# TejasPote/data_diet_distributed

Hardware: AMD Instinct MI355X
Metric: examples scored/sec (whole node), EL2N+GraNd ResNet-18 CIFAR-10, 1/2/4/8 GPU (higher is better)
Workload: dtype fp32 (split MFMA: hi*hi + hi*lo + lo*hi with fp32 accumulation; EL2N forward on f16x3 halves, GraNd forward on f16x3, GraNd backward on bf16x3); 1 GPU; R18/C10 EL2N+GraNd, K checkpoints, global keep-set; arch=resnet18, input=3x32x32 cifar stem, n_examples=50000, checkpoints=10, classes=10, score_batch=128, grand_batch=1024, el2n_chunk=1024, kept=25000, select_by=el2n, pegrad_method=auto, grand_params=conv_linear, passes=sequential, lanes=3, launch_plan=full chunks + short tail, el2n_operands=f16x3

## Files before the change

data_diet_distributed_amd/csrc/dd_conv_kern.h:

```cpp
#pragma once

#ifndef DD_R2_FENCE
#define DD_R2_FENCE 2
#endif
#include "dd_mfma.h"

namespace dd {
namespace conv {

struct Args {
  const float* x;
  const __bf16* wpack;
  const float* bias;
  const float* residual;
  const float* mask_src;
  const float* in_scale;
  const float* in_shift;
  float* y;
  float* stats;
  uint16_t* mask_out;
  const uint16_t* mask_in;
  int64_t B, n_stat;
  int cin, H, cout, op, cp;
  int relu, xf_mask, gsize, tiles_per_group;
// ... 60 lines not shown
  static constexpr int XS = W * 2;
  static constexpr int PLANE = CC * XS;
  static constexpr int ROWP = 3 * 2 * PLANE + (W == 16 ? 128 : W == 8 ? 64 : W == 4 ? 32 : 0);
  static constexpr int IMGP = (RB + 2) * ROWP + (W == 4 ? 192 : 0);
  static constexpr int BUF = E * IMGP;
  static constexpr int LDS = 2 * BUF > BUF + 16384 ? 2 * BUF : BUF + 16384;
  static constexpr int TB = E * RB * W;
  static constexpr int TW = TB / WT;
  static constexpr int NT = TW / 32;
  static constexpr int OB = WO * NA * 32;
  static constexpr int TPR = W / 4;
  static constexpr int NF4 = NR * CC * W / 4;
  static constexpr int NST = (NF4 + 255) / 256;
  static_assert(TW % 32 == 0 && NT >= 1, "a wave must own whole 32-position tiles");
  static_assert(WO * WT == 4, "four waves per workgroup");
};

template <int W, int RB, int E, int NA, int WO, int XF, bool KX1, int EPI = 0, int PW = 0>
__global__ __launch_bounds__(256, NA == 1 ? 2 : 1) void conv3x3_kernel(const Args A) {
  using C = Cfg<W, RB, E, NA, WO>;
  constexpr int NT = C::NT;
  constexpr bool F16 = (EPI & kEpiF16) != 0;
  static_assert(!PW || (XF <= kXfAffine && !KX1 && (EPI & ~kEpiF16) == (kEpiSpec | kEpiStats)),
                "padded-width tiles: the statistics epilogue with an optional BN staging only");
  extern __shared__ __attribute__((aligned(16))) char smem[];
  const int H = A.H, cin = A.cin, cout = A.cout;
  const int64_t B = A.B;
  const float* __restrict__ x = A.x;
  const int WG = PW ? A.wg : W;
  const int HW = H * WG;
// ... 453 lines not shown
      }
    }
    for (; kc + 1 < nchunks; ++kc) chunk(T, kc + 1, true);
    const Tile Tn = has_next ? decode(tile_n) : T;
    chunk(Tn, has_next ? 0 : nchunks - 1, false);
    load_w_taps(Tn.ob32, 0, 0, 3);
    epilogue(T, tile, (g - 1) & 1);
    __syncthreads();
    load_w_taps(Tn.ob32, 0, 3, 6);
    if (!has_next) break;
    tile = tile_n;
    T = Tn;
  }
}

template <int W, int RB, int E, int WO, int XF, bool KX1, int EPI = 0, int PW = 0>
__global__ __launch_bounds__(256, 2) void conv3x3_r2_kernel(const Args A) {
  using C = Cfg<W, RB, E, 1, WO>;
  constexpr int NT = C::NT;
  constexpr bool F16 = (EPI & kEpiF16) != 0;
  static_assert(!PW || (XF <= kXfAffine && !KX1 && (EPI & ~kEpiF16) == (kEpiSpec | kEpiStats)),
                "padded-width tiles: the statistics epilogue with an optional BN staging only");
  extern __shared__ __attribute__((aligned(16))) char smem[];
  const int H = A.H, cin = A.cin, cout = A.cout;
  const int64_t B = A.B;
  const float* __restrict__ x = A.x;
  const int WG = PW ? A.wg : W;
  const int HW = H * WG;
  const int HWP = PW ? A.n_tb * RB * W : HW;
  const int ntiles = A.n_tiles;

  const int tid = threadIdx.x, lane = tid & 63;
  const int wv = __builtin_amdgcn_readfirstlane(tid >> 6);
  const int wo = wv % WO, wt = wv / WO, h = lane >> 5;

  struct Tile {
    int64_t b, grp;
    int tb, o0, y0, xf_base, ob32;
  };
  auto decode = [&](int tile) {
    Tile T;
    int bid = tile;
    const int ob = bid % A.n_ob;
    bid /= A.n_ob;
    T.tb = bid % A.n_tb;
    T.b = (int64_t)(bid / A.n_tb) * E;
    T.o0 = ob * C::OB;
    T.y0 = T.tb * RB;
    T.grp = T.b / A.gsize;
    T.xf_base = (int)(T.grp * cin);
    T.ob32 = (T.o0 >> 5) + wo;
    return T;
  };

  float4 ra[C::NST];
  static_assert(256 % (C::TPR * CC) == 0, "a thread's staged channel must not depend on k");
  float xs = 1.f, xt = 0.f;
  bool va[C::NST];
  float4 rv[C::NST];
  float rs = 1.f, rt = 0.f;
  __amdgpu_buffer_rsrc_t xo_rsrc;
  int xo_base = 0;
  bool xo_tile = false;
  auto load_chunk = [&](const Tile& T, int c0) {
    const int64_t left = (B - T.b) * cin * HW * 4;
    const uint32_t range = (uint32_t)(left < 0x7fffffff ? left : 0x7fffffff);
    const __amdgpu_buffer_rsrc_t xr = buffer_rsrc(x + (size_t)T.b * cin * HW, range);
    const int ubase = c0 * HW * 4;
    __amdgpu_buffer_rsrc_t rr_rsrc;
    if constexpr (XF >= kXfOut) {
      xo_rsrc = buffer_rsrc(A.xout + (size_t)T.b * cin * HW, range);
      xo_base = ubase + (T.y0 - 1) * W * 4;
      xo_tile = T.o0 == 0;
      if constexpr (XF >= kXfOutRes) rr_rsrc = buffer_rsrc(A.xres + (size_t)T.b * cin * HW, range);
    }
#pragma unroll
    for (int k = 0; k < C::NST; ++k) {
      const int q = tid + 256 * k;
      const int x4 = q % C::TPR, c = (q / C::TPR) % CC, sr = q / (C::TPR * CC);
      const int e = sr / (RB + 2), rr = sr - e * (RB + 2);
      const int ir = T.y0 - 1 + rr, cg = c0 + c;
      va[k] = q < C::NF4 && ir >= 0 && ir < H && cg < cin && T.b + e < B &&
              (!PW || x4 * 4 < WG);
      const int irc = ir < 0 ? 0 : (ir >= H ? H - 1 : ir);
      const int xoff = ubase + ((e * cin + c) * HW + irc * WG + x4 * 4) * 4;
      if constexpr (PW == 2) {
        ra[k] = make_float4(
            __builtin_bit_cast(float, __builtin_amdgcn_raw_buffer_load_b32(xr, xoff, 0, 0)),
            __builtin_bit_cast(float, __builtin_amdgcn_raw_buffer_load_b32(xr, xoff + 4, 0, 0)),
            __builtin_bit_cast(float, __builtin_amdgcn_raw_buffer_load_b32(xr, xoff + 8, 0, 0)),
            __builtin_bit_cast(float, __builtin_amdgcn_raw_buffer_load_b32(xr, xoff + 12, 0, 0)));
      } else {
        ra[k] = __builtin_bit_cast(float4, __builtin_amdgcn_raw_buffer_load_b128(xr, xoff, 0, 0));
// ... 5 lines not shown
    }
    if constexpr (XF != kXfNone) {
      const int cg = c0 + (tid / C::TPR) % CC;
      const int xi = T.xf_base + (cg < cin ? cg : cin - 1);
      xs = A.in_scale[xi];
      xt = A.in_shift[xi];
      if constexpr (XF == kXfOutResAff) {
        rs = A.xres_scale[xi];
        rt = A.xres_shift[xi];
      }
    }
  };
  auto store_chunk = [&](int buf) {
    char* base0 = smem + buf * C::BUF;
#pragma unroll
    for (int k = 0; k < C::NST; ++k) {
      const int q = tid + 256 * k;
      if (C::NF4 % 256 != 0 && k == C::NST - 1 && q >= C::NF4) continue;
      const int x4 = q % C::TPR, c = (q / C::TPR) % CC, sr = q / (C::TPR * CC);
      const int se = sr / (RB + 2), rr = sr - se * (RB + 2);
      float4 v = ra[k];
      if constexpr (XF != kXfNone) v = stage_transform<XF>(v, xs, xt, rv[k], rs, rt, A.in_floor);
      v = keep_if(v, va[k]);
      if constexpr (PW == 2) v = keep_cols(v, WG - x4 * 4);
      if constexpr (XF >= kXfOut) {
        const bool wr = xo_tile && va[k] && rr >= 1 && rr <= RB;
        const int off = xo_base + ((se * cin + c) * HW + rr * W + x4 * 4) * 4;
        __builtin_amdgcn_raw_buffer_store_b128(__builtin_bit_cast(uint4v, v), xo_rsrc,
                                               wr ? off : (int)0x80000000, 0, 0);
      }
      uint2 hs[3], ls[3];
      split_shift3<F16>(v, x4 == 0, x4 == C::TPR - 1, hs, ls);
      if constexpr (KX1) {
// ... 57 lines not shown
    floatx16 d = acc[n];
    d = mfma16<F16>(ws[set][kx][0], bb[n][0], d);
    d = mfma16<F16>(ws[set][kx][0], bb[n][1], d);
    d = mfma16<F16>(ws[set][kx][1], bb[n][0], d);
    acc[n] = d;
  };

  auto epilogue = [&](const Tile& T, int tile, int free_buf) {
    const EpiFlags F = epi_flags<EPI>(A);
    const float* __restrict__ bias = A.bias;
    const float* __restrict__ residual = A.residual;
    const float* __restrict__ mask_src = A.mask_src;
    float* __restrict__ y = A.y;
    float* ep = reinterpret_cast<float*>(smem + free_buf * C::BUF) + wv * 1024;
    const int tl = lane & 7, ol = lane >> 3;
    size_t ibase[NT];
    bool vlan[NT];
    float in_stat[NT];
    int ncol[NT];
#pragma unroll
    for (int n = 0; n < NT; ++n) {
      const int tt = wt * C::TW + n * 32 + 4 * tl;
      const int e = tt / (RB * W);
      int t = T.y0 * W + tt % (RB * W);
      bool in_img = true;
      if constexpr (PW) {
        const int rem = tt % (RB * W), row = T.y0 + rem / W, col = rem % W;
        in_img = row < H && col < WG;
        ncol[n] = WG - col;
        t = in_img ? row * WG + col : 0;
// ... 32 lines not shown
      if (F.msrc) {
#pragma unroll
        for (int m = 0; m < NG; ++m) {
          unsigned mb = 0;
#pragma unroll
          for (int k = 0; k < 4; ++k) {
            const float4 mk = *reinterpret_cast<const float4*>(mask_src + ibase[n0 + m] + off[k]);
            mb |= ((mk.x > 0.f ? 1u : 0u) | (mk.y > 0.f ? 2u : 0u) | (mk.z > 0.f ? 4u : 0u) |
                   (mk.w > 0.f ? 8u : 0u)) << (4 * k);
          }
          mbits[m] = mb;
        }
      } else {
#pragma unroll
        for (int m = 0; m < NG; ++m) {
          const size_t fidx = (((size_t)tile * 4 + wv) * NT + n0 + m) * 64 + lane;
          mbits[m] = F.min ? A.mask_in[fidx] : 0xffffu;
        }
      }
#pragma unroll
      for (int m = 0; m < NG; ++m) {
        const int n = n0 + m;
#pragma unroll
        for (int r = 0; r < 16; ++r)
          ep[((r & 3) + 8 * (r >> 2) + 4 * h) * 32 + (lane & 31)] =
              F16 ? acc[n][r] * A.acc_scale : acc[n][r];
        asm volatile("" ::: "memory");
        float4 v[4];
#pragma unroll
        for (int k = 0; k < 4; ++k)
          v[k] = *reinterpret_cast<const float4*>(ep + (8 * k + ol) * 32 + 4 * tl);
// ... 31 lines not shown
#pragma unroll
              for (int j = 0; j < 4; ++j)
                if (j < ncol[n]) y[ibase[n] + off[k] + j] = f[j];
            }
          } else if (vlan[n] && o < cout) {
            store_out4(y + ibase[n] + off[k], f[0], f[1], f[2], f[3]);
          }
          if (F.stats) {
            s_ = sum8(s_);
            q_ = sum8(q_);
            if (tl == 0 && o < cout)
              *reinterpret_cast<float2*>(sp + k * 16 * A.tiles_per_group) = make_float2(s_, q_);
          }
        }
        if (F.mout) {
          const size_t fidx = (((size_t)tile * 4 + wv) * NT + n) * 64 + lane;
          A.mask_out[fidx] = (uint16_t)obits;
        }
      }
    });
  };

  auto chunk = [&](auto Pc, auto W2c, const Tile& T, int c, const Tile& Ts, int ks,
                   const Tile& Tw, int kw) {
    constexpr int P = decltype(Pc)::value;
    load_chunk(Ts, ks * CC);
#if DD_R2_FENCE >= 1
    __builtin_amdgcn_sched_barrier(0);
#endif
    constexpr int T0 = KX1 ? 1 : 0, TS = KX1 ? 3 : 1;
#pragma unroll
// ... 141 lines not shown

template <int W, int RB, int E, int NA, int WO>
struct GoNarrow {
  const Args& a;
  dim3 g;
  hipStream_t st;
  template <int XF, bool KX1, int EPI>
  int run() {
    constexpr auto K = &conv3x3_kernel<W, RB, E, NA, WO, XF, KX1, EPI>;
    lds_attr<K>(Cfg<W, RB, E, NA, WO>::LDS);
    K<<<g, 256, Cfg<W, RB, E, NA, WO>::LDS, st>>>(a);
    DD_CHECK_LAUNCH("dd_conv3x3_forward");
    return DD_OK;
  }
};
template <int W, int RB, int E, int WO>
struct GoR2 {
  static constexpr int LDS = Cfg<W, RB, E, 1, WO>::LDS;
  const Args& a;
  dim3 g;
  hipStream_t st;
  template <int XF, bool KX1, int EPI>
  int run() {
    constexpr auto K = &conv3x3_r2_kernel<W, RB, E, WO, XF, KX1, EPI>;
    lds_attr<K>(LDS);
    K<<<g, 256, LDS, st>>>(a);
    DD_CHECK_LAUNCH("dd_conv3x3_forward");
    return DD_OK;
  }
};

template <int W, int RB, int E, int NA, int WO>
static int launch(Args a, hipStream_t st) {
  using C = Cfg<W, RB, E, NA, WO>;
  DD_REQUIRE(a.H % RB == 0, "dd_conv3x3_forward: H must be a multiple of the row block");
  DD_REQUIRE(a.gsize % E == 0, "dd_conv3x3_forward: group_size %d must be a multiple of %d "
             "(images per tile at %dx%d)", a.gsize, E, a.H, W);
  DD_REQUIRE(a.op % C::OB == 0, "dd_conv3x3_forward: padded outputs %d not a multiple of %d",
             a.op, C::OB);
  a.n_tb = a.H / RB;
  a.n_ob = a.op / C::OB;
  const int64_t ntiles = ceil_div(a.B, E) * a.n_tb * a.n_ob;
  DD_REQUIRE(ntiles < (1ll << 31), "dd_conv3x3_forward: too many tiles");
  a.n_tiles = (int)ntiles;
  const int64_t cap = NA == 2 ? device_cus() : a.cin <= 256 ? 2ll * device_cus() : ntiles;
  const int64_t grid = ntiles < cap ? ntiles : cap;
  GoNarrow<W, RB, E, NA, WO> go{a, dim3((unsigned)grid), st};
  return dispatch_epi<kSpecNarrow<W, RB, E, NA, WO>>(a, go);
}

template <int W, int RB, int E, int WO>
static int launch_r2(Args a, hipStream_t st) {
  using C = Cfg<W, RB, E, 1, WO>;
  static_assert(2 * C::LDS <= 160 * 1024, "r2 tiles run two workgroups per CU");
  DD_REQUIRE(a.H % RB == 0, "dd_conv3x3_forward: H must be a multiple of the row block");
  DD_REQUIRE(a.gsize % E == 0, "dd_conv3x3_forward: group_size %d must be a multiple of %d "
             "(images per tile at %dx%d)", a.gsize, E, a.H, W);
  DD_REQUIRE(a.op % C::OB == 0, "dd_conv3x3_forward: padded outputs %d not a multiple of %d",
             a.op, C::OB);
  a.n_tb = a.H / RB;
  a.n_ob = a.op / C::OB;
  const int64_t ntiles = ceil_div(a.B, E) * a.n_tb * a.n_ob;
  DD_REQUIRE(ntiles < (1ll << 31), "dd_conv3x3_forward: too many tiles");
  a.n_tiles = (int)ntiles;
  const int64_t cap = 2ll * device_cus();
  GoR2<W, RB, E, WO> go{a, dim3((unsigned)(ntiles < cap ? ntiles : cap)), st};
  return dispatch_epi<true, decltype(go), W >= 8>(a, go);
}

template <int W, int RB, int E, int PW, int XF, int EPI>
static int run_pw(const Args& a, dim3 g, hipStream_t st) {
  constexpr auto K = &conv3x3_r2_kernel<W, RB, E, 4, XF, false, EPI, PW>;
  lds_attr<K>(Cfg<W, RB, E, 1, 4>::LDS);
  K<<<g, 256, Cfg<W, RB, E, 1, 4>::LDS, st>>>(a);
  DD_CHECK_LAUNCH("dd_conv3x3_forward");
  return DD_OK;
}
template <int W, int RB, int E, int PW>
static int launch_r2_pw(Args a, hipStream_t st) {
  using C = Cfg<W, RB, E, 1, 4>;
  static_assert(2 * C::LDS <= 160 * 1024, "r2 tiles run two workgroups per CU");
// ... 44 lines not shown
  a.n_ob = a.op / C::OB;
  const int64_t ntiles = ceil_div(a.B, E) * a.n_tb * a.n_ob;
  DD_REQUIRE(ntiles < (1ll << 31), "dd_conv3x3_forward: too many tiles");
  a.n_tiles = (int)ntiles;
  const int64_t cap = (int64_t)(160 * 1024 / C::LDS) * device_cus();
  const dim3 g((unsigned)(ntiles < cap ? ntiles : cap));
  const bool xf = a.xf_mask != 0;
  if (a.f16)
    return xf ? run_pw_narrow<W, RB, E, PW, kXfAffine, kE_Stats | kEpiF16>(a, g, st)
              : run_pw_narrow<W, RB, E, PW, kXfNone, kE_Stats | kEpiF16>(a, g, st);
  return xf ? run_pw_narrow<W, RB, E, PW, kXfAffine, kE_Stats>(a, g, st)
            : run_pw_narrow<W, RB, E, PW, kXfNone, kE_Stats>(a, g, st);
}

int dispatch_r2(int w, int key, const Args& a, hipStream_t st);
int dispatch_small(int w, int key, const Args& a, hipStream_t st);
int dispatch_pw(int w, int pw, const Args& a, hipStream_t st);

}
}
```

data_diet_distributed_amd/csrc/dd_conv_r2.hip:

```cpp
#include "dd_conv_kern.h"

namespace dd {
namespace conv {

int dispatch_r2(int w, int k, const Args& a, hipStream_t st) {
  if (w == 16 && k == 8000 + 100 + 10 + 4) return launch_r2<16, 8, 1, 4>(a, st);
  if (w == 8 && k == 8000 + 200 + 10 + 4) return launch_r2<8, 8, 2, 4>(a, st);
  if (w == 4 && k == 4000 + 800 + 10 + 4) return launch_r2<4, 4, 8, 4>(a, st);
  set_error("dd_conv3x3_forward: no r2 kernel for tile key %d at w=%d", k, w);
  return DD_EINVAL;
}

}
}
```

data_diet_distributed_amd/csrc/dd_down.hip:

```cpp
#include "dd_mfma.h"

#include <stdlib.h>

namespace dd {
namespace down {

using namespace conv;

template <int WO, int RB, int E>
struct DCfg {
  static constexpr int SR = 2 * RB + 1;
  static constexpr int NR = E * SR;
  static constexpr int WI = 2 * WO;
  static constexpr int XS = WO * 2;
  static constexpr int PLANE = CC * XS;
  static constexpr int ROWP = 3 * 2 * PLANE + (WO == 16 ? 64 : WO == 8 ? 32 : WO == 4 ? 16 : 0);
  static constexpr int IMGP = SR * ROWP + (WO == 4 ? 240 : 0);
  static constexpr int BUF = E * IMGP;
  static constexpr int TB = E * RB * WO;
  static constexpr int TPR = WI / 8;
  static constexpr int NF8 = NR * CC * WI / 8;
  static constexpr int NST = (NF8 + 255) / 256;
  static constexpr int TPR4 = WI / 4;
  static constexpr int NF4 = NR * CC * WI / 4;
  static constexpr int NST4 = (NF4 + 255) / 256;
  static constexpr int TAILB = (NF8 % 256 != 0 || NF4 % 256 != 0) ? 6 * PLANE + 512 : 0;
  static constexpr int LDS = 2 * BUF + TAILB;
  static_assert(TB == 64, "two 32-position t tiles per workgroup");
  static_assert(WO % 4 == 0, "transposed reads take 4 consecutive columns");
  static_assert(BUF >= 4 * 4096, "the epilogue's four 4 KB transpose blocks live in a buffer");
};

struct Out {
  float* y;
  const float* bias;
  float* stats;
  int relu;
  float scale;
};

struct FwdArgs {
  const float* x;
  const __bf16* w3;
  const __bf16* ws;
  Out main, sc;
  int64_t B, n_stat;
  int cin, HO, cout, nob32;
  int gsize, tiles_per_group, n_tb, n_ob, n_tiles;
  int xcd;
  int wog;
  const float* in_scale;
  const float* in_shift;
  const float* xres;
};

constexpr int kXmNone = 0, kXmAffine = 1, kXmUnit = 3;

template <int WO, int RB, int E, bool SC, bool PT, int WA, int EPI = 0, int XM = 0,
          bool F16 = false, int PW = 0>
__global__ __launch_bounds__(256, 2) void down_fwd_kernel(const FwdArgs A) {
  using C = DCfg<WO, RB, E>;
  constexpr int NT = WA == 4 ? 2 : 1;
  constexpr bool S8 = WO >= 8;
  static_assert(!PW || (!SC && S8 && E == 1 && XM != kXmUnit && EPI == 0),
                "padded-width heads: the plain EL2N statistics launch");
  extern __shared__ __attribute__((aligned(16))) char smem[];
  const int HO = A.HO, HI = 2 * HO, cin = A.cin, cout = A.cout;
  const int64_t B = A.B;
  const int WOG = PW ? A.wog : WO, WIG = 2 * WOG;
  const int HWI = HI * WIG, HWO = HO * WOG;
  const int ntiles = A.n_tiles;

  const int tid = threadIdx.x, lane = tid & 63;
  const int wv = WA == 4 ? __builtin_amdgcn_readfirstlane(tid >> 6) : tid >> 6;
  const int wo = WA == 4 ? wv : wv & 1, wt = WA == 4 ? 0 : wv >> 1, h = lane >> 5;

  struct Tile {
    int64_t b, grp;
    int tb, y0, o_w, ob32;
  };
  auto decode = [&](int tile) {
    Tile T;
    int bid = tile;
    const int ob = bid % A.n_ob;
    bid /= A.n_ob;
    T.tb = bid % A.n_tb;
    T.b = (int64_t)(bid / A.n_tb) * E;
    T.y0 = T.tb * RB;
    T.grp = T.b / A.gsize;
    T.o_w = ob * 32 * WA + wo * 32;
    T.ob32 = T.o_w >> 5;
    return T;
  };

  const float* __restrict__ x = A.x;
  float4 ra4[S8 ? 1 : C::NST4];
  bool va4[S8 ? 1 : C::NST4];
  static_assert(256 % (C::TPR4 * CC) == 0 && 256 % (C::TPR * CC) == 0,
                "a thread's staged channel must not depend on the round");
  float xs = 1.f, xt = 0.f;
  float4 rr4[(S8 || XM != kXmUnit) ? 1 : C::NST4];
  float4 rr8[(S8 && XM == kXmUnit) ? C::NST : 1][2];
  auto load_affine = [&](const Tile& T, int c0, int tpr) {
    if constexpr (XM != kXmNone) {
      const int cg = c0 + (tid / tpr) % CC;
      const int xi = (int)(T.grp * cin) + (cg < cin ? cg : cin - 1);
      xs = A.in_scale[xi];
      xt = A.in_shift[xi];
    }
  };
  auto xform = [&](float4 v, float4 r) {
    if constexpr (XM == kXmNone) {
      return v;
    } else {
      v = make_float4(fmaf(v.x, xs, xt), fmaf(v.y, xs, xt), fmaf(v.z, xs, xt), fmaf(v.w, xs, xt));
      if constexpr (XM == kXmUnit) v = make_float4(v.x + r.x, v.y + r.y, v.z + r.z, v.w + r.w);
      return make_float4(nmax(v.x, 0.f), nmax(v.y, 0.f), nmax(v.z, 0.f), nmax(v.w, 0.f));
    }
  };
  auto load_chunk4 = [&](const Tile& T, int c0) {
#pragma unroll
    for (int k = 0; k < C::NST4; ++k) {
      const int q = tid + 256 * k;
      const int x4 = q % C::TPR4, c = (q / C::TPR4) % CC, sr = q / (C::TPR4 * CC);
      const int e = sr / C::SR, rr = sr - e * C::SR;
      const int ir = 2 * T.y0 - 1 + rr, cg = c0 + c;
      const bool ve = T.b + e < B;
      va4[k] = q < C::NF4 && ir >= 0 && ir < HI && cg < cin && ve;
      const int irc = ir < 0 ? 0 : (ir >= HI ? HI - 1 : ir);
      const int cgc = cg < cin ? cg : cin - 1;
      const int64_t bc = ve ? T.b + e : B - 1;
      const size_t ofs = ((size_t)bc * cin + cgc) * HWI + irc * C::WI + x4 * 4;
      ra4[k] = *reinterpret_cast<const float4*>(x + ofs);
      if constexpr (!S8 && XM == kXmUnit) rr4[k] = *reinterpret_cast<const float4*>(A.xres + ofs);
    }
    load_affine(T, c0, C::TPR4);
  };
  auto store_chunk4 = [&](int buf) {
    char* base0 = smem + buf * C::BUF;
#pragma unroll
    for (int k = 0; k < C::NST4; ++k) {
      const int q = tid + 256 * k;
      const bool tail = C::NF4 % 256 != 0 && k == C::NST4 - 1 && q >= C::NF4;
      const int x4 = q % C::TPR4, c = (q / C::TPR4) % CC, sr = q / (C::TPR4 * CC);
      float4 rk = make_float4(0.f, 0.f, 0.f, 0.f);
      if constexpr (!S8 && XM == kXmUnit) rk = rr4[k];
      const float4 v = keep_if(xform(ra4[k], rk), va4[k]);
      float left = lane_prev<C::TPR4>(v.w);
      if (x4 == 0) left = 0.f;
      const float f[3][2] = {{left, v.y}, {v.x, v.z}, {v.y, v.w}};
#pragma unroll
      for (int kx = 0; kx < 3; ++kx) {
        __bf16 h0, l0, h1, l1;
        split16<F16>(f[kx][0], h0, l0);
        split16<F16>(f[kx][1], h1, l1);
        const int se = sr / C::SR, rr = sr - se * C::SR;
        char* p = tail ? smem + 2 * C::BUF + (kx * 2) * C::PLANE + lane * 4
                       : base0 + se * C::IMGP + rr * C::ROWP + (kx * 2) * C::PLANE + c * C::XS +
                             x4 * 4;
        typedef __bf16 bf16x2 __attribute__((ext_vector_type(2)));
        *reinterpret_cast<bf16x2*>(p) = bf16x2{h0, h1};
        *reinterpret_cast<bf16x2*>(p + C::PLANE) = bf16x2{l0, l1};
      }
    }
  };

  float4 ra[S8 ? C::NST : 1][2];
  bool va[S8 ? C::NST : 1];
  auto load_chunk8 = [&](const Tile& T, int c0) {
#pragma unroll
    for (int k = 0; k < C::NST; ++k) {
      const int q = tid + 256 * k;
      const int x8 = q % C::TPR, c = (q / C::TPR) % CC, sr = q / (C::TPR * CC);
      const int e = sr / C::SR, rr = sr - e * C::SR;
      const int ir = 2 * T.y0 - 1 + rr, cg = c0 + c;
      const bool ve = T.b + e < B;
      va[k] = q < C::NF8 && ir >= 0 && ir < HI && cg < cin && ve && (!PW || x8 * 8 < WIG);
      const int irc = ir < 0 ? 0 : (ir >= HI ? HI - 1 : ir);
      const int cgc = cg < cin ? cg : cin - 1;
      const int64_t bc = ve ? T.b + e : B - 1;
      const int col = PW && x8 * 8 >= WIG ? 0 : x8 * 8;
      const size_t ofs = ((size_t)bc * cin + cgc) * HWI + irc * WIG + col;
      if constexpr (PW == 3) {
        float v[8];
#pragma unroll
        for (int j = 0; j < 8; ++j) v[j] = x[ofs + (col + j < WIG ? j : 0)];
        ra[k][0] = make_float4(v[0], v[1], v[2], v[3]);
// ... 1 lines not shown
      } else {
        ra[k][0] = *reinterpret_cast<const float4*>(x + ofs);
        ra[k][1] = *reinterpret_cast<const float4*>(x + ofs + (!PW || col + 4 < WIG ? 4 : 0));
      }
      if constexpr (S8 && XM == kXmUnit) {
        rr8[k][0] = *reinterpret_cast<const float4*>(A.xres + ofs);
        rr8[k][1] = *reinterpret_cast<const float4*>(A.xres + ofs + 4);
      }
    }
    load_affine(T, c0, C::TPR);
  };
  auto store_chunk8 = [&](int buf) {
    char* base0 = smem + buf * C::BUF;
#pragma unroll
    for (int k = 0; k < C::NST; ++k) {
      const int q = tid + 256 * k;
      const bool tail = C::NF8 % 256 != 0 && k == C::NST - 1 && q >= C::NF8;
      const int x8 = q % C::TPR, c = (q / C::TPR) % CC, sr = q / (C::TPR * CC);
      float4 r0 = make_float4(0.f, 0.f, 0.f, 0.f), r1 = r0;
      if constexpr (S8 && XM == kXmUnit) {
        r0 = rr8[k][0];
        r1 = rr8[k][1];
      }
      float4 v0 = keep_if(xform(ra[k][0], r0), va[k]), v1 = keep_if(xform(ra[k][1], r1), va[k]);
      if constexpr (PW != 0) {
        v0 = keep_cols(v0, WIG - x8 * 8);
        v1 = keep_cols(v1, WIG - x8 * 8 - 4);
      }
      float left = C::TPR > 1 ? lane_prev<C::TPR>(v1.w) : 0.f;
      if (x8 == 0) left = 0.f;
      const float f[9] = {left, v0.x, v0.y, v0.z, v0.w, v1.x, v1.y, v1.z, v1.w};
      __bf16 hv[9], lv[9];
// ... 196 lines not shown
            acc_s[n] = s_;
          }
          if constexpr (t + 1 < 9) rb(t + 1, n);
        }
        if (wload) {
          load_w_taps(Tp.ob32, kn, t, 1);
          if constexpr (t == 4) load_w_sc(Tp.ob32, kn);
        }
        if constexpr (t == 6) store_chunk(cur ^ 1);
        __builtin_amdgcn_sched_barrier(0);
      });
      __syncthreads();
      ++g;
    };
    auto chunk = [&](const Tile& Tp, int kn, bool wload) {
      if constexpr (WA == 4) {
        chunk4(Tp, kn, wload);
        return;
      }
      const int cur = g & 1;
      load_chunk(Tp, kn * CC);
      const char* base = smem + cur * C::BUF;
      bf16x8 b0[3][2], b1[3][2];
      read_b(base, 0, b0);
      __builtin_amdgcn_sched_barrier(0);
      read_b(base, 1, b1);
      mfma_row(0, b0);
      if (wload) load_w_taps(Tp.ob32, kn, 0, 3);
#pragma unroll
      for (int i = 0; i < 3; ++i) {
        __builtin_amdgcn_sched_group_barrier(0x008, 1, 0);
// ... 26 lines not shown
#pragma unroll
      for (int i = 0; i < 9; ++i) {
        __builtin_amdgcn_sched_group_barrier(0x008, 1, 2);
        __builtin_amdgcn_sched_group_barrier(0x002, 5, 2);
        __builtin_amdgcn_sched_group_barrier(0x080, 1, 2);
      }
      __builtin_amdgcn_sched_barrier(0);
      __syncthreads();
      ++g;
    };
    for (int kc = 0; kc + 1 < nchunks; ++kc) chunk(T, kc + 1, true);
    {
      const Tile Tn = has_next ? decode(tile_n) : T;
      chunk(Tn, has_next ? 0 : nchunks - 1, false);
    }
    char* ep_buf = smem + ((g - 1) & 1) * C::BUF;
#pragma unroll
    for (int n = 0; n < NT; ++n) {
      epilogue(T, acc[n], A.main, T.o_w, ep_buf, wt + n, std::true_type{});
      if constexpr (SC) epilogue(T, acc_s[n], A.sc, T.o_w, ep_buf, wt + n, std::false_type{});
    }
    if constexpr (!PT) break;
    __syncthreads();
    const int tile_w = has_next ? tile_n : tile;
    T = decode(tile_w);
    load_w_ordered(T.ob32, 0);
    if (!has_next) break;
    tile = tile_n;
  }
}

// ... 460 lines not shown
    const int no = tflip ? cin : cout, nc = tflip ? cout : cin;
    float v = 0.f;
    if (o < no && c < nc) v = tflip ? w[(size_t)c * cin + o] : w[(size_t)o * cin + c];
    v *= scale;
    __bf16 hi, lo;
    if (f16)
      split16<true>(v, hi, lo);
    else
      split16<false>(v, hi, lo);
    out[i] = pr == 0 ? hi : lo;
  }
}

template <int WO, int RB, int E, bool SC, int WA, int EPI = 0, int XM = 0, bool F16 = false>
static int launch_fwd(FwdArgs a, hipStream_t st) {
  using C = DCfg<WO, RB, E>;
  static bool attr = false;
  if (!attr) {
    (void)hipFuncSetAttribute(
        reinterpret_cast<const void*>(&down_fwd_kernel<WO, RB, E, SC, false, WA, EPI, XM, F16>),
        hipFuncAttributeMaxDynamicSharedMemorySize, C::LDS);
    (void)hipFuncSetAttribute(
        reinterpret_cast<const void*>(&down_fwd_kernel<WO, RB, E, SC, true, WA, EPI, XM, F16>),
        hipFuncAttributeMaxDynamicSharedMemorySize, C::LDS);
    attr = true;
  }
  DD_REQUIRE(a.HO % RB == 0, "dd_down_forward: HO must be a multiple of the row block");
  DD_REQUIRE(a.gsize % E == 0, "dd_down_forward: group_size %d must be a multiple of %d",
             a.gsize, E);
  a.n_tb = a.HO / RB;
  a.n_ob = (int)ceil_div(a.cout, 32 * WA);
  a.tiles_per_group = (a.gsize / E) * a.n_tb * 2;
  const int64_t ntiles = ceil_div(a.B, E) * a.n_tb * a.n_ob;
  DD_REQUIRE(ntiles < (1ll << 31), "dd_down_forward: too many tiles");
  a.n_tiles = (int)ntiles;
  const bool pt = a.cin <= 64;
  const int64_t cap = pt ? 2ll * device_cus() : ntiles;
  const int64_t grid = ntiles < cap ? ntiles : cap;
  if (pt)
    down_fwd_kernel<WO, RB, E, SC, true, WA, EPI, XM, F16>
        <<<(unsigned)grid, 256, C::LDS, st>>>(a);
  else
    down_fwd_kernel<WO, RB, E, SC, false, WA, EPI, XM, F16>
        <<<(unsigned)grid, 256, C::LDS, st>>>(a);
  DD_CHECK_LAUNCH("dd_down_forward");
  return DD_OK;
}

template <int WO, int RB, int PW, int XM, bool F16>
static int launch_fwd_pw(FwdArgs a, hipStream_t st) {
  using C = DCfg<WO, RB, 1>;
  constexpr auto K = &down_fwd_kernel<WO, RB, 1, false, false, 4, 0, XM, F16, PW>;
  static bool attr = false;
  if (!attr) {
    (void)hipFuncSetAttribute(reinterpret_cast<const void*>(K),
                              hipFuncAttributeMaxDynamicSharedMemorySize, C::LDS);
    attr = true;
  }
  a.n_tb = (a.HO + RB - 1) / RB;
// ... 5 lines not shown
  K<<<(unsigned)ntiles, 256, C::LDS, st>>>(a);
  DD_CHECK_LAUNCH("dd_down_forward");
  return DD_OK;
}

static int fwd_epi(const Out& m, const Out& s) {
  static const int f = env_int("DD_DOWN_EPI", 1);
  if (f == 0 || !s.y) return 0;
  if (!m.bias && !m.relu && m.stats && !s.bias && !s.relu && s.stats) return 1;
  if (m.bias && m.relu && !m.stats && s.bias && !s.relu && !s.stats) return 2;
  return 0;
}
static int fwd_wa(int cout) {
  static const int f = env_int("DD_DOWN_WA", 4);
  return f == 4 && conv::pad_to(cout, 64) % 128 == 0 ? 4 : 2;
}

template <int WO, int RB, int E, bool SC>
static int launch_bwd(BwdArgs a, hipStream_t st) {
  using C = UCfg<WO, RB, E, SC>;
  static bool attr = false;
  if (!attr) {
    (void)hipFuncSetAttribute(reinterpret_cast<const void*>(&down_bwd_kernel<WO, RB, E, SC>),
                              hipFuncAttributeMaxDynamicSharedMemorySize, C::LDS);
    attr = true;
  }
  DD_REQUIRE(a.HO % RB == 0, "dd_down_backward: HO must be a multiple of the row block");
  a.n_tb = a.HO / RB;
  a.n_ob = (int)ceil_div(a.cin, 64);
  const int64_t grid = ceil_div(a.B, E) * a.n_tb * a.n_ob;
// ... 173 lines not shown
               "dd_down_forward_unit_input: the unit form needs the fused shortcut and "
               "statistics on both outputs");
    DD_REQUIRE(!in_scale || xres || !sc,
               "dd_down_forward_unit_input: BN + ReLU staging without a shortcut only");
#define DD_DOWN_F(WO_, RB_, E_, WA_)                                                          \
    if (xres) return down::launch_fwd<WO_, RB_, E_, true, WA_, 1, down::kXmUnit, true>(a, st); \
    if (in_scale) return down::launch_fwd<WO_, RB_, E_, false, WA_, 0, down::kXmAffine, true>(a, st); \
    if (sc && epi == 1) return down::launch_fwd<WO_, RB_, E_, true, WA_, 1, 0, true>(a, st); \
    if (sc && epi == 2) return down::launch_fwd<WO_, RB_, E_, true, WA_, 2, 0, true>(a, st); \
    if (sc) return down::launch_fwd<WO_, RB_, E_, true, WA_, 0, 0, true>(a, st);           \
    return down::launch_fwd<WO_, RB_, E_, false, WA_, 0, 0, true>(a, st);
#define DD_DOWN_FW(WO_, RB_, E_) \
    if (wa == 4) { DD_DOWN_F(WO_, RB_, E_, 4) } else { DD_DOWN_F(WO_, RB_, E_, 2) }
    if (wo == 32) { DD_DOWN_FW(32, 2, 1) }
    if (wo == 16) { DD_DOWN_FW(16, 4, 1) }
    if (wo == 8) { DD_DOWN_FW(8, 8, 1) }
    DD_DOWN_FW(4, 4, 4)
#undef DD_DOWN_FW
#undef DD_DOWN_F
  }
  if (in_scale) {
    const int wa = down::fwd_wa(cout);
#define DD_DOWN_X(WO_, RB_, E_)                                                          \
    if (xres) {                                                                          \
      DD_REQUIRE(sc && down::fwd_epi(a.main, a.sc) == 1,                                 \
                 "dd_down_forward_unit_input: the unit form needs the fused shortcut and " \
                 "statistics on both outputs");                                          \
      return wa == 4 ? down::launch_fwd<WO_, RB_, E_, true, 4, 1, down::kXmUnit>(a, st) \
                     : down::launch_fwd<WO_, RB_, E_, true, 2, 1, down::kXmUnit>(a, st); \
    }                                                                                    \
    DD_REQUIRE(!sc, "dd_down_forward_unit_input: BN + ReLU staging without a shortcut only"); \
    return wa == 4 ? down::launch_fwd<WO_, RB_, E_, false, 4, 0, down::kXmAffine>(a, st) \
                   : down::launch_fwd<WO_, RB_, E_, false, 2, 0, down::kXmAffine>(a, st);
    if (wo == 32) { DD_DOWN_X(32, 2, 1) }
    if (wo == 16) { DD_DOWN_X(16, 4, 1) }
    if (wo == 8) { DD_DOWN_X(8, 8, 1) }
    DD_DOWN_X(4, 4, 4)
#undef DD_DOWN_X
  }
  const int wa = down::fwd_wa(cout);
  const int epi = down::fwd_epi(a.main, a.sc);
#define DD_DOWN_SC(WO_, RB_, E_, WA_)                                                  \
  (epi == 1   ? down::launch_fwd<WO_, RB_, E_, true, WA_, 1>(a, st)                \
   : epi == 2 ? down::launch_fwd<WO_, RB_, E_, true, WA_, 2>(a, st)                \
              : down::launch_fwd<WO_, RB_, E_, true, WA_, 0>(a, st))
#define DD_DOWN(WO_, RB_, E_)                                                    \
  return wa == 4 ? (sc ? DD_DOWN_SC(WO_, RB_, E_, 4)                             \
                       : down::launch_fwd<WO_, RB_, E_, false, 4>(a, st))        \
                 : (sc ? DD_DOWN_SC(WO_, RB_, E_, 2)                             \
                       : down::launch_fwd<WO_, RB_, E_, false, 2>(a, st))
  if (wo == 32) DD_DOWN(32, 2, 1);
  if (wo == 16) DD_DOWN(16, 4, 1);
  if (wo == 8) DD_DOWN(8, 8, 1);
  DD_DOWN(4, 4, 4);
#undef DD_DOWN
#undef DD_DOWN_SC
}

int dd_down_forward(const float* x, int64_t B, int32_t cin, int32_t ho, int32_t wo,
                    const void* packed3x3, const void* packed1x1, int32_t cout,
                    const float* bias, int32_t relu, float* stats, float* y,
                    const float* bias_sc, int32_t relu_sc, float* stats_sc, float* y_sc,
                    int32_t group_size, int64_t n_stat, int32_t operands, float acc_scale,
                    float acc_scale_sc, void* stream) {
  clear_error();
  return down_forward_impl(x, B, cin, ho, wo, packed3x3, packed1x1, cout, bias, relu, stats, y,
                           bias_sc, relu_sc, stats_sc, y_sc, group_size, n_stat, nullptr,
// ... 81 lines not shown
```

Before: 8930 examples/s.

## Add 8-wave workgroup variants for small-spatial r2 conv and downsample kernels

Adds 512-thread, eight-wave forms of the r2 3x3 convolution kernel (8x8 and 4x4 maps) and the downsample forward kernel. Each workgroup now spans 256 output channels instead of 128, so one staged input tile is reused across twice as many outputs. Occupancy drops to one workgroup per CU with a larger LDS budget. The mask index math is generalised to the new output blocking. Both forms are on by default through environment flags when cout padding allows it, which risks lower latency hiding and fewer workgroups on the small late layers.

```diff
diff --git a/data_diet_distributed_amd/csrc/dd_conv_kern.h b/data_diet_distributed_amd/csrc/dd_conv_kern.h
--- a/data_diet_distributed_amd/csrc/dd_conv_kern.h
+++ b/data_diet_distributed_amd/csrc/dd_conv_kern.h
@@ -98,6 +98,14 @@
   static constexpr int NST = (NF4 + 255) / 256;
   static_assert(TW % 32 == 0 && NT >= 1, "a wave must own whole 32-position tiles");
   static_assert(WO * WT == 4, "four waves per workgroup");
+};
+
+template <int W, int RB, int E>
+struct R2W8 {
+  using C = Cfg<W, RB, E, 1, 4>;
+  static constexpr int OB = 8 * 32;
+  static constexpr int NST = (C::NF4 + 511) / 512;
+  static constexpr int LDS = 2 * C::BUF > C::BUF + 32768 ? 2 * C::BUF : C::BUF + 32768;
 };
 
 template <int W, int RB, int E, int NA, int WO, int XF, bool KX1, int EPI = 0, int PW = 0>
@@ -581,10 +589,17 @@
   }
 }
 
-template <int W, int RB, int E, int WO, int XF, bool KX1, int EPI = 0, int PW = 0>
-__global__ __launch_bounds__(256, 2) void conv3x3_r2_kernel(const Args A) {
+template <int W, int RB, int E, int WO, int XF, bool KX1, int EPI = 0, int PW = 0, int NW = 4>
+__global__ __launch_bounds__(NW * 64, NW == 4 ? 2 : 1) void conv3x3_r2_kernel(const Args A) {
   using C = Cfg<W, RB, E, 1, WO>;
+  using C8 = R2W8<W, RB, E>;
   constexpr int NT = C::NT;
+  constexpr int NTH = NW * 64;
+  constexpr int WOK = NW == 8 ? 8 : WO;
+  constexpr int OBK = NW == 8 ? C8::OB : C::OB;
+  constexpr int NST = NW == 8 ? C8::NST : C::NST;
+  static_assert(NW == 4 || (NW == 8 && WO == 4 && !PW && !KX1),
+                "the 8-wave form: the native 8x8 / 4x4 tiles, eight waves along o");
   constexpr bool F16 = (EPI & kEpiF16) != 0;
   static_assert(!PW || (XF <= kXfAffine && !KX1 && (EPI & ~kEpiF16) == (kEpiSpec | kEpiStats)),
                 "padded-width tiles: the statistics epilogue with an optional BN staging only");
@@ -599,7 +614,7 @@
 
   const int tid = threadIdx.x, lane = tid & 63;
   const int wv = __builtin_amdgcn_readfirstlane(tid >> 6);
-  const int wo = wv % WO, wt = wv / WO, h = lane >> 5;
+  const int wo = wv % WOK, wt = wv / WOK, h = lane >> 5;
 
   struct Tile {
     int64_t b, grp;
@@ -612,7 +627,7 @@
     bid /= A.n_ob;
     T.tb = bid % A.n_tb;
     T.b = (int64_t)(bid / A.n_tb) * E;
-    T.o0 = ob * C::OB;
+    T.o0 = ob * OBK;
     T.y0 = T.tb * RB;
     T.grp = T.b / A.gsize;
     T.xf_base = (int)(T.grp * cin);
@@ -620,11 +635,11 @@
     return T;
   };
 
-  float4 ra[C::NST];
-  static_assert(256 % (C::TPR * CC) == 0, "a thread's staged channel must not depend on k");
+  float4 ra[NST];
+  static_assert(NTH % (C::TPR * CC) == 0, "a thread's staged channel must not depend on k");
   float xs = 1.f, xt = 0.f;
-  bool va[C::NST];
-  float4 rv[C::NST];
+  bool va[NST];
+  float4 rv[NST];
   float rs = 1.f, rt = 0.f;
   __amdgpu_buffer_rsrc_t xo_rsrc;
   int xo_base = 0;
@@ -642,8 +657,8 @@
       if constexpr (XF >= kXfOutRes) rr_rsrc = buffer_rsrc(A.xres + (size_t)T.b * cin * HW, range);
     }
 #pragma unroll
-    for (int k = 0; k < C::NST; ++k) {
-      const int q = tid + 256 * k;
+    for (int k = 0; k < NST; ++k) {
+      const int q = tid + NTH * k;
       const int x4 = q % C::TPR, c = (q / C::TPR) % CC, sr = q / (C::TPR * CC);
       const int e = sr / (RB + 2), rr = sr - e * (RB + 2);
       const int ir = T.y0 - 1 + rr, cg = c0 + c;
@@ -679,9 +694,9 @@
   auto store_chunk = [&](int buf) {
     char* base0 = smem + buf * C::BUF;
 #pragma unroll
-    for (int k = 0; k < C::NST; ++k) {
-      const int q = tid + 256 * k;
-      if (C::NF4 % 256 != 0 && k == C::NST - 1 && q >= C::NF4) continue;
+    for (int k = 0; k < NST; ++k) {
+      const int q = tid + NTH * k;
+      if (C::NF4 % NTH != 0 && k == NST - 1 && q >= C::NF4) continue;
       const int x4 = q % C::TPR, c = (q / C::TPR) % CC, sr = q / (C::TPR * CC);
       const int se = sr / (RB + 2), rr = sr - se * (RB + 2);
       float4 v = ra[k];
@@ -769,6 +784,8 @@
     float* __restrict__ y = A.y;
     float* ep = reinterpret_cast<float*>(smem + free_buf * C::BUF) + wv * 1024;
     const int tl = lane & 7, ol = lane >> 3;
+    const size_t fb32 = NW == 4 ? (size_t)tile * 4 + wv
+                                : (size_t)(tile / A.n_ob) * nob32 + T.ob32;
     size_t ibase[NT];
     bool vlan[NT];
     float in_stat[NT];
@@ -831,7 +848,7 @@
       } else {
 #pragma unroll
         for (int m = 0; m < NG; ++m) {
-          const size_t fidx = (((size_t)tile * 4 + wv) * NT + n0 + m) * 64 + lane;
+          const size_t fidx = ((size_t)fb32 * NT + n0 + m) * 64 + lane;
           mbits[m] = F.min ? A.mask_in[fidx] : 0xffffu;
         }
       }
@@ -893,7 +910,7 @@
           }
         }
         if (F.mout) {
-          const size_t fidx = (((size_t)tile * 4 + wv) * NT + n) * 64 + lane;
+          const size_t fidx = ((size_t)fb32 * NT + n) * 64 + lane;
           A.mask_out[fidx] = (uint16_t)obits;
         }
       }
@@ -1065,17 +1082,26 @@
     return DD_OK;
   }
 };
-template <int W, int RB, int E, int WO>
+template <int W, int RB, int E, int WO, int NW = 4>
 struct GoR2 {
-  static constexpr int LDS = Cfg<W, RB, E, 1, WO>::LDS;
+  static constexpr int LDS = NW == 8 ? R2W8<W, RB, E>::LDS : Cfg<W, RB, E, 1, WO>::LDS;
   const Args& a;
   dim3 g;
   hipStream_t st;
   template <int XF, bool KX1, int EPI>
   int run() {
-    constexpr auto K = &conv3x3_r2_kernel<W, RB, E, WO, XF, KX1, EPI>;
+    if constexpr (NW == 8 && KX1) {
+      set_error("dd_conv3x3_forward: the 8-wave tiles have no stem layout");
+      return DD_EINVAL;
+    } else {
+      return run_<XF, KX1, EPI>();
+    }
+  }
+  template <int XF, bool KX1, int EPI>
+  int run_() {
+    constexpr auto K = &conv3x3_r2_kernel<W, RB, E, WO, XF, KX1, EPI, 0, NW>;
     lds_attr<K>(LDS);
-    K<<<g, 256, LDS, st>>>(a);
+    K<<<g, NW * 64, LDS, st>>>(a);
     DD_CHECK_LAUNCH("dd_conv3x3_forward");
     return DD_OK;
   }
@@ -1100,22 +1126,24 @@
   return dispatch_epi<kSpecNarrow<W, RB, E, NA, WO>>(a, go);
 }
 
-template <int W, int RB, int E, int WO>
+template <int W, int RB, int E, int WO, int NW = 4>
 static int launch_r2(Args a, hipStream_t st) {
   using C = Cfg<W, RB, E, 1, WO>;
-  static_assert(2 * C::LDS <= 160 * 1024, "r2 tiles run two workgroups per CU");
+  constexpr int OB = NW == 8 ? R2W8<W, RB, E>::OB : C::OB;
+  static_assert((NW == 8 ? 1 : 2) * GoR2<W, RB, E, WO, NW>::LDS <= 160 * 1024,
+                "r2 tiles run two 4-wave workgroups, or one 8-wave workgroup, per CU");
   DD_REQUIRE(a.H % RB == 0, "dd_conv3x3_forward: H must be a multiple of the row block");
   DD_REQUIRE(a.gsize % E == 0, "dd_conv3x3_forward: group_size %d must be a multiple of %d "
              "(images per tile at %dx%d)", a.gsize, E, a.H, W);
-  DD_REQUIRE(a.op % C::OB == 0, "dd_conv3x3_forward: padded outputs %d not a multiple of %d",
-             a.op, C::OB);
+  DD_REQUIRE(a.op % OB == 0, "dd_conv3x3_forward: padded outputs %d not a multiple of %d",
+             a.op, OB);
   a.n_tb = a.H / RB;
-  a.n_ob = a.op / C::OB;
+  a.n_ob = a.op / OB;
   const int64_t ntiles = ceil_div(a.B, E) * a.n_tb * a.n_ob;
   DD_REQUIRE(ntiles < (1ll << 31), "dd_conv3x3_forward: too many tiles");
   a.n_tiles = (int)ntiles;
-  const int64_t cap = 2ll * device_cus();
-  GoR2<W, RB, E, WO> go{a, dim3((unsigned)(ntiles < cap ? ntiles : cap)), st};
+  const int64_t cap = (NW == 8 ? 1ll : 2ll) * device_cus();
+  GoR2<W, RB, E, WO, NW> go{a, dim3((unsigned)(ntiles < cap ? ntiles : cap)), st};
   return dispatch_epi<true, decltype(go), W >= 8>(a, go);
 }
 
@@ -1190,6 +1218,7 @@
 }
 
 int dispatch_r2(int w, int key, const Args& a, hipStream_t st);
+int dispatch_r2_w8(int w, int key, const Args& a, hipStream_t st);
 int dispatch_small(int w, int key, const Args& a, hipStream_t st);
 int dispatch_pw(int w, int pw, const Args& a, hipStream_t st);
 
diff --git a/data_diet_distributed_amd/csrc/dd_conv_r2.hip b/data_diet_distributed_amd/csrc/dd_conv_r2.hip
--- a/data_diet_distributed_amd/csrc/dd_conv_r2.hip
+++ b/data_diet_distributed_amd/csrc/dd_conv_r2.hip
@@ -3,7 +3,12 @@
 namespace dd {
 namespace conv {
 
+static bool use_w8(int w, const Args& a) {
+  return (w == 8 || w == 4) && a.op % 256 == 0 && !a.kx1 && env_int("DD_CONV_W8", 1) != 0;
+}
+
 int dispatch_r2(int w, int k, const Args& a, hipStream_t st) {
+  if (use_w8(w, a)) return dispatch_r2_w8(w, k, a, st);
   if (w == 16 && k == 8000 + 100 + 10 + 4) return launch_r2<16, 8, 1, 4>(a, st);
   if (w == 8 && k == 8000 + 200 + 10 + 4) return launch_r2<8, 8, 2, 4>(a, st);
   if (w == 4 && k == 4000 + 800 + 10 + 4) return launch_r2<4, 4, 8, 4>(a, st);
diff --git a/data_diet_distributed_amd/csrc/dd_conv_r2w8.hip b/data_diet_distributed_amd/csrc/dd_conv_r2w8.hip
--- /dev/null
+++ b/data_diet_distributed_amd/csrc/dd_conv_r2w8.hip
@@ -0,0 +1,14 @@
+#include "dd_conv_kern.h"
+
+namespace dd {
+namespace conv {
+
+int dispatch_r2_w8(int w, int k, const Args& a, hipStream_t st) {
+  if (w == 8 && k == 8000 + 200 + 10 + 4) return launch_r2<8, 8, 2, 4, 8>(a, st);
+  if (w == 4 && k == 4000 + 800 + 10 + 4) return launch_r2<4, 4, 8, 4, 8>(a, st);
+  set_error("dd_conv3x3_forward: no 8-wave r2 kernel for tile key %d at w=%d", k, w);
+  return DD_EINVAL;
+}
+
+}
+}
diff --git a/data_diet_distributed_amd/csrc/dd_down.hip b/data_diet_distributed_amd/csrc/dd_down.hip
--- a/data_diet_distributed_amd/csrc/dd_down.hip
+++ b/data_diet_distributed_amd/csrc/dd_down.hip
@@ -7,7 +7,7 @@
 
 using namespace conv;
 
-template <int WO, int RB, int E>
+template <int WO, int RB, int E, int NTH = 256>
 struct DCfg {
   static constexpr int SR = 2 * RB + 1;
   static constexpr int NR = E * SR;
@@ -20,15 +20,16 @@
   static constexpr int TB = E * RB * WO;
   static constexpr int TPR = WI / 8;
   static constexpr int NF8 = NR * CC * WI / 8;
-  static constexpr int NST = (NF8 + 255) / 256;
+  static constexpr int NST = (NF8 + NTH - 1) / NTH;
   static constexpr int TPR4 = WI / 4;
   static constexpr int NF4 = NR * CC * WI / 4;
-  static constexpr int NST4 = (NF4 + 255) / 256;
-  static constexpr int TAILB = (NF8 % 256 != 0 || NF4 % 256 != 0) ? 6 * PLANE + 512 : 0;
+  static constexpr int NST4 = (NF4 + NTH - 1) / NTH;
+  static constexpr int TAILB = (NF8 % NTH != 0 || NF4 % NTH != 0) ? 6 * PLANE + 512 : 0;
   static constexpr int LDS = 2 * BUF + TAILB;
   static_assert(TB == 64, "two 32-position t tiles per workgroup");
   static_assert(WO % 4 == 0, "transposed reads take 4 consecutive columns");
   static_assert(BUF >= 4 * 4096, "the epilogue's four 4 KB transpose blocks live in a buffer");
+  static_assert(NTH == 256 || 2 * BUF >= 8 * 4096, "the 8-wave form's eight blocks span both");
 };
 
 struct Out {
@@ -58,9 +59,12 @@
 
 template <int WO, int RB, int E, bool SC, bool PT, int WA, int EPI = 0, int XM = 0,
           bool F16 = false, int PW = 0>
-__global__ __launch_bounds__(256, 2) void down_fwd_kernel(const FwdArgs A) {
-  using C = DCfg<WO, RB, E>;
-  constexpr int NT = WA == 4 ? 2 : 1;
+__global__ __launch_bounds__(WA == 8 ? 512 : 256, WA == 8 ? 1 : 2) void down_fwd_kernel(
+    const FwdArgs A) {
+  constexpr int NTH = WA == 8 ? 512 : 256;
+  using C = DCfg<WO, RB, E, NTH>;
+  constexpr int NT = WA >= 4 ? 2 : 1;
+  static_assert(WA != 8 || (!PT && !PW), "the 8-wave form: one tile per workgroup, native widths");
   constexpr bool S8 = WO >= 8;
   static_assert(!PW || (!SC && S8 && E == 1 && XM != kXmUnit && EPI == 0),
                 "padded-width heads: the plain EL2N statistics launch");
@@ -72,8 +76,8 @@
   const int ntiles = A.n_tiles;
 
   const int tid = threadIdx.x, lane = tid & 63;
-  const int wv = WA == 4 ? __builtin_amdgcn_readfirstlane(tid >> 6) : tid >> 6;
-  const int wo = WA == 4 ? wv : wv & 1, wt = WA == 4 ? 0 : wv >> 1, h = lane >> 5;
+  const int wv = WA >= 4 ? __builtin_amdgcn_readfirstlane(tid >> 6) : tid >> 6;
+  const int wo = WA >= 4 ? wv : wv & 1, wt = WA >= 4 ? 0 : wv >> 1, h = lane >> 5;
 
   struct Tile {
     int64_t b, grp;
@@ -96,7 +100,7 @@
   const float* __restrict__ x = A.x;
   float4 ra4[S8 ? 1 : C::NST4];
   bool va4[S8 ? 1 : C::NST4];
-  static_assert(256 % (C::TPR4 * CC) == 0 && 256 % (C::TPR * CC) == 0,
+  static_assert(NTH % (C::TPR4 * CC) == 0 && NTH % (C::TPR * CC) == 0,
                 "a thread's staged channel must not depend on the round");
   float xs = 1.f, xt = 0.f;
   float4 rr4[(S8 || XM != kXmUnit) ? 1 : C::NST4];
@@ -121,7 +125,7 @@
   auto load_chunk4 = [&](const Tile& T, int c0) {
 #pragma unroll
     for (int k = 0; k < C::NST4; ++k) {
-      const int q = tid + 256 * k;
+      const int q = tid + NTH * k;
       const int x4 = q % C::TPR4, c = (q / C::TPR4) % CC, sr = q / (C::TPR4 * CC);
       const int e = sr / C::SR, rr = sr - e * C::SR;
       const int ir = 2 * T.y0 - 1 + rr, cg = c0 + c;
@@ -140,8 +144,8 @@
     char* base0 = smem + buf * C::BUF;
 #pragma unroll
     for (int k = 0; k < C::NST4; ++k) {
-      const int q = tid + 256 * k;
-      const bool tail = C::NF4 % 256 != 0 && k == C::NST4 - 1 && q >= C::NF4;
+      const int q = tid + NTH * k;
+      const bool tail = C::NF4 % NTH != 0 && k == C::NST4 - 1 && q >= C::NF4;
       const int x4 = q % C::TPR4, c = (q / C::TPR4) % CC, sr = q / (C::TPR4 * CC);
       float4 rk = make_float4(0.f, 0.f, 0.f, 0.f);
       if constexpr (!S8 && XM == kXmUnit) rk = rr4[k];
@@ -170,7 +174,7 @@
   auto load_chunk8 = [&](const Tile& T, int c0) {
 #pragma unroll
     for (int k = 0; k < C::NST; ++k) {
-      const int q = tid + 256 * k;
+      const int q = tid + NTH * k;
       const int x8 = q % C::TPR, c = (q / C::TPR) % CC, sr = q / (C::TPR * CC);
       const int e = sr / C::SR, rr = sr - e * C::SR;
       const int ir = 2 * T.y0 - 1 + rr, cg = c0 + c;
@@ -202,8 +206,8 @@
     char* base0 = smem + buf * C::BUF;
 #pragma unroll
     for (int k = 0; k < C::NST; ++k) {
-      const int q = tid + 256 * k;
-      const bool tail = C::NF8 % 256 != 0 && k == C::NST - 1 && q >= C::NF8;
+      const int q = tid + NTH * k;
+      const bool tail = C::NF8 % NTH != 0 && k == C::NST - 1 && q >= C::NF8;
       const int x8 = q % C::TPR, c = (q / C::TPR) % CC, sr = q / (C::TPR * CC);
       float4 r0 = make_float4(0.f, 0.f, 0.f, 0.f), r1 = r0;
       if constexpr (S8 && XM == kXmUnit) {
@@ -430,7 +434,7 @@
       ++g;
     };
     auto chunk = [&](const Tile& Tp, int kn, bool wload) {
-      if constexpr (WA == 4) {
+      if constexpr (WA >= 4) {
         chunk4(Tp, kn, wload);
         return;
       }
@@ -487,7 +491,7 @@
       const Tile Tn = has_next ? decode(tile_n) : T;
       chunk(Tn, has_next ? 0 : nchunks - 1, false);
     }
-    char* ep_buf = smem + ((g - 1) & 1) * C::BUF;
+    char* ep_buf = WA == 8 ? smem : smem + ((g - 1) & 1) * C::BUF;
 #pragma unroll
     for (int n = 0; n < NT; ++n) {
       epilogue(T, acc[n], A.main, T.o_w, ep_buf, wt + n, std::true_type{});
@@ -978,15 +982,18 @@
 
 template <int WO, int RB, int E, bool SC, int WA, int EPI = 0, int XM = 0, bool F16 = false>
 static int launch_fwd(FwdArgs a, hipStream_t st) {
-  using C = DCfg<WO, RB, E>;
+  constexpr int NTH = WA == 8 ? 512 : 256;
+  using C = DCfg<WO, RB, E, NTH>;
+  static_assert((WA == 8 ? 1 : 2) * C::LDS <= 160 * 1024, "LDS of the resident workgroups");
   static bool attr = false;
   if (!attr) {
     (void)hipFuncSetAttribute(
         reinterpret_cast<const void*>(&down_fwd_kernel<WO, RB, E, SC, false, WA, EPI, XM, F16>),
         hipFuncAttributeMaxDynamicSharedMemorySize, C::LDS);
-    (void)hipFuncSetAttribute(
-        reinterpret_cast<const void*>(&down_fwd_kernel<WO, RB, E, SC, true, WA, EPI, XM, F16>),
-        hipFuncAttributeMaxDynamicSharedMemorySize, C::LDS);
+    if constexpr (WA != 8)
+      (void)hipFuncSetAttribute(
+          reinterpret_cast<const void*>(&down_fwd_kernel<WO, RB, E, SC, true, WA, EPI, XM, F16>),
+          hipFuncAttributeMaxDynamicSharedMemorySize, C::LDS);
     attr = true;
   }
   DD_REQUIRE(a.HO % RB == 0, "dd_down_forward: HO must be a multiple of the row block");
@@ -1001,12 +1008,17 @@
   const bool pt = a.cin <= 64;
   const int64_t cap = pt ? 2ll * device_cus() : ntiles;
   const int64_t grid = ntiles < cap ? ntiles : cap;
-  if (pt)
+  if constexpr (WA == 8) {
+    DD_REQUIRE(!pt, "dd_down_forward: the 8-wave form needs cin > 64");
+    down_fwd_kernel<WO, RB, E, SC, false, WA, EPI, XM, F16>
+        <<<(unsigned)grid, NTH, C::LDS, st>>>(a);
+  } else if (pt) {
     down_fwd_kernel<WO, RB, E, SC, true, WA, EPI, XM, F16>
         <<<(unsigned)grid, 256, C::LDS, st>>>(a);
-  else
+  } else {
     down_fwd_kernel<WO, RB, E, SC, false, WA, EPI, XM, F16>
         <<<(unsigned)grid, 256, C::LDS, st>>>(a);
+  }
   DD_CHECK_LAUNCH("dd_down_forward");
   return DD_OK;
 }
@@ -1042,6 +1054,12 @@
 static int fwd_wa(int cout) {
   static const int f = env_int("DD_DOWN_WA", 4);
   return f == 4 && conv::pad_to(cout, 64) % 128 == 0 ? 4 : 2;
+}
+static int fwd_wa8(int wa, int cin, int cout, int wo, bool staged) {
+  return wa == 4 && (wo == 4 || (wo == 8 && staged)) && cin > 64 &&
+                 conv::pad_to(cout, 64) % 256 == 0 && env_int("DD_DOWN_W8", 1) != 0
+             ? 8
+             : wa;
 }
 
 template <int WO, int RB, int E, bool SC>
@@ -1245,6 +1263,13 @@
     if (wa == 4) { DD_DOWN_F(WO_, RB_, E_, 4) } else { DD_DOWN_F(WO_, RB_, E_, 2) }
     if (wo == 32) { DD_DOWN_FW(32, 2, 1) }
     if (wo == 16) { DD_DOWN_FW(16, 4, 1) }
+    if (down::fwd_wa8(wa, cin, cout, wo, in_scale != nullptr) == 8) {
+      if (wo == 8) {
+        if (xres) return down::launch_fwd<8, 8, 1, true, 8, 1, down::kXmUnit, true>(a, st);
+        return down::launch_fwd<8, 8, 1, false, 8, 0, down::kXmAffine, true>(a, st);
+      }
+      DD_DOWN_F(4, 4, 4, 8)
+    }
     if (wo == 8) { DD_DOWN_FW(8, 8, 1) }
     DD_DOWN_FW(4, 4, 4)
 #undef DD_DOWN_FW
@@ -1265,6 +1290,20 @@
                    : down::launch_fwd<WO_, RB_, E_, false, 2, 0, down::kXmAffine>(a, st);
     if (wo == 32) { DD_DOWN_X(32, 2, 1) }
     if (wo == 16) { DD_DOWN_X(16, 4, 1) }
+    if (down::fwd_wa8(wa, cin, cout, wo, true) == 8) {
+#define DD_DOWN_X8(WO_, RB_, E_)                                                         \
+      if (xres) {                                                                        \
+        DD_REQUIRE(sc && down::fwd_epi(a.main, a.sc) == 1,                               \
+                   "dd_down_forward_unit_input: the unit form needs the fused shortcut and " \
+                   "statistics on both outputs");                                        \
+        return down::launch_fwd<WO_, RB_, E_, true, 8, 1, down::kXmUnit>(a, st);         \
+      }                                                                                  \
+      DD_REQUIRE(!sc, "dd_down_forward_unit_input: BN + ReLU staging without a shortcut only"); \
+      return down::launch_fwd<WO_, RB_, E_, false, 8, 0, down::kXmAffine>(a, st);
+      if (wo == 8) { DD_DOWN_X8(8, 8, 1) }
+      DD_DOWN_X8(4, 4, 4)
+#undef DD_DOWN_X8
+    }
     if (wo == 8) { DD_DOWN_X(8, 8, 1) }
     DD_DOWN_X(4, 4, 4)
 #undef DD_DOWN_X
@@ -1282,6 +1321,8 @@
                        : down::launch_fwd<WO_, RB_, E_, false, 2>(a, st))
   if (wo == 32) DD_DOWN(32, 2, 1);
   if (wo == 16) DD_DOWN(16, 4, 1);
+  if (down::fwd_wa8(wa, cin, cout, wo, false) == 8)
+    return sc ? DD_DOWN_SC(4, 4, 4, 8) : down::launch_fwd<4, 4, 4, false, 8>(a, st);
   if (wo == 8) DD_DOWN(8, 8, 1);
   DD_DOWN(4, 4, 4);
 #undef DD_DOWN
```

New measurement: 8979 examples/s, median of 6. About the same (+0.5%).
